# AlessioSam/LADiff

Hardware: AMD Instinct MI355X
Metric: motions/sec (196-frame, 50-step DDIM, bs128) (higher is better)
Workload: dtype f16x3+f32; 1 GPU; headline:ddim50_cfg7.5_b128_f196_c263_humanml3d; prompts_per_gpu=128, global_batch=128, frames=196, scheduler=ddim, denoising_steps=50, parallelism=dp1, loop=persistent pipeline kernel (16-row blocks x 86)

## Files before the change

### ladiff_amd/csrc/dec_mlp.hip

```cpp
#include <mutex>
#include "model.h"
#include "tile_mma.h"

namespace ladiff {

namespace {

constexpr int MLP_NS = 8;
constexpr int MLP_GRP = 4;
constexpr int MLP_STAGE = 16384;
constexpr int MLP_LDS = MLP_NS * MLP_STAGE + FF * 4 + 5 * D * 4;

typedef unsigned u32x4_m __attribute__((ext_vector_type(4)));

struct MlpArgs {
    const float* xs;
    const float* x;
    const float* w1;
    const float* b1;
    const float* w2;
    const float* b2;
    const float* g3; const float* be3;
    const float* g4; const float* be4;
    float* y; float* ys;
    int M;
};

__device__ __forceinline__ int pi_row(int p) { const int j = p >> 4, n = p & 15; return 32 * (j >> 1) + 8 * (n >> 2) + 4 * (j & 1) + (n & 3); }

template <int N> __device__ __forceinline__ void wait_vm() { asm volatile("s_waitcnt vmcnt(%0)" ::"n"(N) : "memory"); }
template <int OFF>
__device__ __forceinline__ void fetch16(u32x4_m& v, unsigned addr) {
    asm volatile("ds_read_b128 %0, %1 offset:%2" : "=v"(v) : "v"(addr), "n"(OFF) : "memory");
}
template <int OFF>
__device__ __forceinline__ void fetch16_keep(u32x4_m& v, unsigned addr) {
    asm volatile("ds_read_b128 %0, %1 offset:%2" : "+v"(v) : "v"(addr), "n"(OFF) : "memory");
}
template <int N>
__device__ __forceinline__ void wait_lgkm(u32x4_m& a, u32x4_m& b, u32x4_m& c, u32x4_m& d) {
    asm volatile("s_waitcnt lgkmcnt(%4)" : "+v"(a), "+v"(b), "+v"(c), "+v"(d) : "n"(N));
}
__device__ __forceinline__ s16x8 as_bf(const u32x4_m v) { return __builtin_bit_cast(s16x8, v); }

}

template <int NW, int RT, int DIAG = 0>
__global__ __launch_bounds__(64 * NW, NW / 4) void dec_mlp_kernel(const MlpArgs p) {
    constexpr int NT = 64 * NW, RW = 16 * RT, BM = RW * NW, PPW = 16 / NW;
    extern __shared__ __attribute__((aligned(1024))) char lds[];
    float* const b1s = reinterpret_cast<float*>(lds + MLP_NS * MLP_STAGE);
    const int tid = threadIdx.x, lane = tid & 63;
    const int wave = __builtin_amdgcn_readfirstlane(tid >> 6);
    const int frow = lane & 15, fk = lane >> 4;
    const int M = p.M;
    int myrow[RT]; bool live[RT];
#pragma unroll
    for (int rt = 0; rt < RT; ++rt) {
        myrow[rt] = blockIdx.x * BM + RW * wave + 16 * rt + frow;
        live[rt] = myrow[rt] < M;
        myrow[rt] = live[rt] ? myrow[rt] : M - 1;
    }

    s16x8 xh[RT][8], xl[RT][8];
#pragma unroll
    for (int rt = 0; rt < RT; ++rt) {
        const char* xr = reinterpret_cast<const char*>(p.xs) + (size_t)myrow[rt] * 1024 + fk * 16;
#pragma unroll
        for (int s = 0; s < 8; ++s) {
            xh[rt][s] = *reinterpret_cast<const s16x8*>(xr + (s >> 1) * 256 + (s & 1) * 64);
            xl[rt][s] = *reinterpret_cast<const s16x8*>(xr + (s >> 1) * 256 + (s & 1) * 64 + 128);
        }
    }
    for (int i = tid; i < FF / 4; i += NT) st4(b1s + 4 * i, ld4(p.b1 + 4 * i));
    float* const prm = b1s + FF;
    for (int i = tid; i < 5 * D / 4; i += NT) {
        const int which = i / (D / 4), c4 = i % (D / 4);
        const float* src = which == 0 ? p.b2 : which == 1 ? p.g3 : which == 2 ? p.be3 : which == 3 ? p.g4 : p.be4;
        if (src != nullptr) st4(prm + 4 * i, ld4(src + 4 * c4));
    }

    const int cs = (lane & 7) ^ ((lane >> 4) & 3) ^ (4 * (wave & 1));
    const int koff = (cs < 4 ? cs * 4 : 32 + (cs - 4) * 4);
    int src[PPW];
#pragma unroll
    for (int i = 0; i < PPW; ++i) src[i] = pi_row(8 * (wave + NW * i) + (lane >> 3));
    char* const dma_dst = lds + (8 * wave) * 128;
    auto issue = [&](int hs, auto uc, auto slotc, auto ic) __attribute__((always_inline)) {
        constexpr int u = decltype(uc)::value, slot = decltype(slotc)::value, i = decltype(ic)::value;
        const float* base; int ldw, n0, kb, half;
        const int hsv = hs < 0 ? 0 : hs;
        if constexpr (u < 8) { base = p.w1; ldw = D; n0 = 128 * hsv; kb = u >> 1; half = u & 1; }
        else { constexpr int v = u - 8, c = v >> 1; base = p.w2; ldw = FF; n0 = 128 * (v & 1); kb = 2 * hsv + (c >> 1); half = c & 1; }
        const float* s0 = base + (size_t)(n0 + src[i]) * ldw + kb * 64 + half * 16 + koff;
        if constexpr (DIAG == 1) { if (hs >= 0) return; }
        __builtin_amdgcn_global_load_lds(s0, (__attribute__((address_space(3))) void*)(dma_dst + slot * MLP_STAGE + 8 * NW * i * 128), 16, 0, 0);
    };

    const int sw = (frow >> 1) & 7;
    const unsigned rd_hi = lds_addr(lds) + frow * 128 + ((fk ^ sw) << 4);
    const unsigned rd_lo = lds_addr(lds) + frow * 128 + (((4 + fk) ^ sw) << 4);
    const unsigned rd_hi2 = rd_hi + 4 * MLP_STAGE, rd_lo2 = rd_lo + 4 * MLP_STAGE;

    f32x4 hacc[RT][8], oacc[RT][16];
    s16x8 hh[RT][4], hl[RT][4];
#pragma unroll
    for (int rt = 0; rt < RT; ++rt)
#pragma unroll
        for (int j = 0; j < 16; ++j) oacc[rt][j] = f32x4{0.f, 0.f, 0.f, 0.f};

    u32x4_m wt[4][2];
    u32x4_m dummy[4][2];
    if constexpr (DIAG == 3 || DIAG == 6 || DIAG == 7) {
#pragma unroll
        for (int i = 0; i < 4; ++i) { asm volatile("" : "=v"(wt[i][0])); asm volatile("" : "=v"(wt[i][1])); asm volatile("" : "=v"(dummy[i][0])); asm volatile("" : "=v"(dummy[i][1])); }
    }
    auto fetch_tile = [&](auto slotc, auto jc) __attribute__((always_inline)) {
        constexpr int slot = decltype(slotc)::value, j = decltype(jc)::value;
        if constexpr (DIAG == 3) return;
        const unsigned ah = slot < 4 ? rd_hi : rd_hi2, al = slot < 4 ? rd_lo : rd_lo2;
        constexpr int so = (slot & 3) * MLP_STAGE;
        if constexpr (DIAG == 6) { fetch16_keep<so + j * 2048>(dummy[j & 3][0], ah); fetch16_keep<so + j * 2048>(dummy[j & 3][1], al); return; }
        fetch16<so + j * 2048>(wt[j & 3][0], ah); fetch16<so + j * 2048>(wt[j & 3][1], al);
    };
    auto stage_mma = [&](auto slotc, auto& acc, auto j0c, const s16x8 (&bh)[RT], const s16x8 (&bl)[RT], auto&& between, auto&& next) __attribute__((always_inline)) {
        constexpr int slot = decltype(slotc)::value, J0 = decltype(j0c)::value;
        static_for<8>([&](auto jc) {
            constexpr int j = decltype(jc)::value, cur = j & 3;
            next(jc);
            if constexpr (DIAG != 3 && DIAG != 6) asm volatile("s_waitcnt lgkmcnt(4)" : "+v"(wt[cur][0]), "+v"(wt[cur][1]));
            __builtin_amdgcn_sched_barrier(0);
            static_for<3 * RT>([&](auto mc) {
                constexpr int m = decltype(mc)::value, prod = m / RT, rt = m % RT;
                if constexpr (DIAG == 7) {
                    acc[rt][J0 + j] = MFMA16_S16(as_bf(dummy[cur][prod == 1]), prod == 0 ? bl[rt] : bh[rt], acc[rt][J0 + j], 0, 0, 0);
                } else if constexpr (DIAG != 2) {
                    if constexpr (prod == 0) acc[rt][J0 + j] = MFMA16_S16(as_bf(wt[cur][0]), bl[rt], acc[rt][J0 + j], 0, 0, 0);
                    else if constexpr (prod == 1) acc[rt][J0 + j] = MFMA16_S16(as_bf(wt[cur][1]), bh[rt], acc[rt][J0 + j], 0, 0, 0);
                    else acc[rt][J0 + j] = MFMA16_S16(as_bf(wt[cur][0]), bh[rt], acc[rt][J0 + j], 0, 0, 0);
                }
                if constexpr (m == 0) {
                    __builtin_amdgcn_sched_barrier(0);
                    if constexpr (j + 3 < 8) fetch_tile(slotc, IntC<j + 3>{});
                    else fetch_tile(IntC<(slot + 1) % MLP_NS>{}, IntC<j + 3 - 8>{});
                    __builtin_amdgcn_sched_barrier(0);
                }
            });
            if constexpr (DIAG == 2) acc[0][J0 + j][0] += __builtin_bit_cast(float, wt[cur][0][0]) + __builtin_bit_cast(float, wt[cur][1][1]);
            __builtin_amdgcn_sched_barrier(0);
            if constexpr (j & 1) between(IntC<j / 2>{});
        });
    };

    static_for<MLP_GRP>([&](auto uc) {
        constexpr int u = decltype(uc)::value;
        static_for<PPW>([&](auto ic) { issue(DIAG == 1 ? -1 : 0, IntC<u>{}, IntC<u>{}, ic); });
    });
    __syncthreads();
    auto landed = [&]() __attribute__((always_inline)) {
        wait_vm<0>();
        __builtin_amdgcn_s_barrier();
    };
    landed();
    static_for<PPW>([&](auto ic) { issue(DIAG == 1 ? -1 : 0, IntC<MLP_GRP>{}, IntC<MLP_GRP>{}, ic); });
    static_for<3>([&](auto jc) { fetch_tile(IntC<0>{}, jc); });
    constexpr int H = PPW / 2;
#pragma unroll 1
    for (int hs = 0; hs < 8; ++hs) {
        static_for<16>([&](auto uc) {
            constexpr int u = decltype(uc)::value, slot = u % MLP_NS, r = u % MLP_GRP;
            auto batch_pieces = [&](auto aheadc, auto halfc) __attribute__((always_inline)) {
                constexpr int ahead = decltype(aheadc)::value, half = decltype(halfc)::value;
                constexpr int ut = (u + ahead) % 16, slot_t = (u + ahead) % MLP_NS;
                const int hs_t = (hs + (u + ahead >= 16 ? 1 : 0)) & 7;
                static_for<H>([&](auto ic) { issue(hs_t, IntC<ut>{}, IntC<slot_t>{}, IntC<H * half + decltype(ic)::value>{}); });
            };
            auto between = [&](auto gc) __attribute__((always_inline)) {
                constexpr int g = decltype(gc)::value;
                if constexpr (r == 3 && g >= 2) batch_pieces(IntC<5>{}, IntC<g - 2>{});
                else if constexpr (r == 0 && g < 2) batch_pieces(IntC<5>{}, IntC<g>{});
                else if constexpr (r == 0 && g >= 2) batch_pieces(IntC<6>{}, IntC<g - 2>{});
                else if constexpr (r == 1 && g < 2) batch_pieces(IntC<6>{}, IntC<g>{});
            };
            auto next = [&](auto jc) __attribute__((always_inline)) {
                constexpr int j = decltype(jc)::value;
                if constexpr (r == 3 && j == 5) landed();
                else if constexpr (r == 0 && j == 5) __builtin_amdgcn_s_barrier();
            };
            if constexpr (u < 8) {
                if constexpr (u == 0) {
#pragma unroll
                    for (int rt = 0; rt < RT; ++rt)
#pragma unroll
                        for (int j = 0; j < 8; ++j) hacc[rt][j] = f32x4{0.f, 0.f, 0.f, 0.f};
                }
                s16x8 bh[RT], bl[RT];
#pragma unroll
                for (int rt = 0; rt < RT; ++rt) { bh[rt] = xh[rt][u]; bl[rt] = xl[rt][u]; }
                stage_mma(IntC<slot>{}, hacc, IntC<0>{}, bh, bl, between, next);
            } else {
                constexpr int v = u - 8, c = v >> 1, nh = v & 1;
                if constexpr (nh == 0) {
                    const f32x4 ba = ld4(b1s + 128 * hs + 32 * c + 8 * fk), bb = ld4(b1s + 128 * hs + 32 * c + 8 * fk + 4);
#pragma unroll
                    for (int rt = 0; rt < RT; ++rt) {
                        f32x4 va, vb;
#pragma unroll
                        for (int e = 0; e < 4; ++e) {
                            if constexpr (DIAG == 4) { va[e] = hacc[rt][2 * c][e] + ba[e]; vb[e] = hacc[rt][2 * c + 1][e] + bb[e]; }
                            else { va[e] = gelu_erf(hacc[rt][2 * c][e] + ba[e]); vb[e] = gelu_erf(hacc[rt][2 * c + 1][e] + bb[e]); }
                        }
                        split8(va, vb, hh[rt][c], hl[rt][c]);
                    }
                }
                s16x8 bh[RT], bl[RT];
#pragma unroll
                for (int rt = 0; rt < RT; ++rt) { bh[rt] = hh[rt][c]; bl[rt] = hl[rt][c]; }
                stage_mma(IntC<slot>{}, oacc, IntC<8 * nh>{}, bh, bl, between, next);
            }
        });
    }
    wait_vm<0>();
    if constexpr (DIAG == 6) {
        wait_lgkm<0>(dummy[0][0], dummy[0][1], dummy[1][0], dummy[1][1]);
        wait_lgkm<0>(dummy[2][0], dummy[2][1], dummy[3][0], dummy[3][1]);
    } else if constexpr (DIAG != 3) {
        wait_lgkm<0>(wt[0][0], wt[0][1], wt[1][0], wt[1][1]);
        wait_lgkm<0>(wt[2][0], wt[2][1], wt[3][0], wt[3][1]);
    }

    if constexpr (DIAG == 5) {
        float s = 0.f;
#pragma unroll
        for (int rt = 0; rt < RT; ++rt)
#pragma unroll
            for (int jj = 0; jj < 16; ++jj) s += oacc[rt][jj][0] + oacc[rt][jj][1] + oacc[rt][jj][2] + oacc[rt][jj][3];
        if (live[0] && p.y != nullptr) p.y[(size_t)myrow[0] * D + fk] = s;
        return;
    }
    __syncthreads();
    char* const stg = lds + wave * 16384;
#pragma unroll
    for (int rt = 0; rt < RT; ++rt) {
        const size_t rbase = (size_t)myrow[rt] * D;
        f32x4 (&v)[16] = oacc[rt];
        float s = 0.f;
#pragma unroll
        for (int jj = 0; jj < 16; ++jj) {
            const int col = 32 * (jj >> 1) + 8 * fk + 4 * (jj & 1);
            const f32x4 bv = ld4(prm + col), rv = ld4(p.x + rbase + col);
#pragma unroll
            for (int e = 0; e < 4; ++e) { v[jj][e] = v[jj][e] + bv[e] + rv[e]; }
            s += (v[jj][0] + v[jj][1]) + (v[jj][2] + v[jj][3]);
        }
#pragma unroll
        for (int pass = 0; pass < 2; ++pass) {
            if (pass == 1 && p.g4 == nullptr) break;
            const float* gp = prm + (pass == 0 ? 1 : 3) * D;
            const float* bp = prm + (pass == 0 ? 2 : 4) * D;
            if (pass == 1) {
                s = 0.f;
#pragma unroll
                for (int jj = 0; jj < 16; ++jj) s += (v[jj][0] + v[jj][1]) + (v[jj][2] + v[jj][3]);
            }
            s += __shfl_xor(s, 16, 64); s += __shfl_xor(s, 32, 64);
            const float mean = s * (1.f / 256.f);
            float q = 0.f;
#pragma unroll
            for (int jj = 0; jj < 16; ++jj)
#pragma unroll
                for (int e = 0; e < 4; ++e) { const float d = v[jj][e] - mean; q = fmaf(d, d, q); }
            q += __shfl_xor(q, 16, 64); q += __shfl_xor(q, 32, 64);
            const float rstd = rsqrtf(q * (1.f / 256.f) + LN_EPS);
#pragma unroll
            for (int jj = 0; jj < 16; ++jj) {
                const int col = 32 * (jj >> 1) + 8 * fk + 4 * (jj & 1);
                const f32x4 ga = ld4(gp + col), be = ld4(bp + col);
#pragma unroll
                for (int e = 0; e < 4; ++e) v[jj][e] = (v[jj][e] - mean) * rstd * ga[e] + be[e];
            }
        }
#pragma unroll
        for (int jj = 0; jj < 16; ++jj) {
            const int ch = 8 * (jj >> 1) + 2 * fk + (jj & 1);
            *reinterpret_cast<f32x4*>(stg + frow * 1024 + ((ch ^ frow) << 4)) = v[jj];
        }
        const int row0 = blockIdx.x * BM + RW * wave + 16 * rt;
#pragma unroll
        for (int r = 0; r < 16; ++r) {
            const f32x4 o = *reinterpret_cast<const f32x4*>(stg + r * 1024 + ((lane ^ r) << 4));
            if (row0 + r < M) {
                if (p.y != nullptr) st4(p.y + (size_t)(row0 + r) * D + 4 * lane, o);
                if (p.ys != nullptr) store_split4(p.ys + (size_t)(row0 + r) * D, 4 * lane, o);
            }
        }
    }
}

std::atomic<int> g_mlp_variant{0};

int dec_mlp_prepare() {
    static std::mutex mu;
    static bool attr_set[64] = {};
    int dev = 0;
    LADIFF_HIP(hipGetDevice(&dev));
    if (dev < 0 || dev >= 64) return LADIFF_ERR_ARG;
    std::lock_guard<std::mutex> lock(mu);
    if (!attr_set[dev]) {
        const void* k[3] = {reinterpret_cast<const void*>(dec_mlp_kernel<4, 2>), reinterpret_cast<const void*>(dec_mlp_kernel<8, 1>),
                            reinterpret_cast<const void*>(dec_mlp_kernel<4, 1>)};
        for (int i = 0; i < 3; ++i) LADIFF_HIP(hipFuncSetAttribute(k[i], hipFuncAttributeMaxDynamicSharedMemorySize, MLP_LDS));
#ifdef LADIFF_STAMPS
        const void* d[7] = {reinterpret_cast<const void*>(dec_mlp_kernel<4, 2, 1>), reinterpret_cast<const void*>(dec_mlp_kernel<4, 2, 2>),
                            reinterpret_cast<const void*>(dec_mlp_kernel<4, 2, 3>), reinterpret_cast<const void*>(dec_mlp_kernel<4, 2, 4>),
                            reinterpret_cast<const void*>(dec_mlp_kernel<4, 2, 5>), reinterpret_cast<const void*>(dec_mlp_kernel<4, 2, 6>),
                            reinterpret_cast<const void*>(dec_mlp_kernel<4, 2, 7>)};
        for (int i = 0; i < 7; ++i) LADIFF_HIP(hipFuncSetAttribute(d[i], hipFuncAttributeMaxDynamicSharedMemorySize, MLP_LDS));
#endif
        attr_set[dev] = true;
    }
    return 0;
}
int dec_mlp_min_rows() { return 10000; }

int launch_dec_mlp(const float* xs, const float* x, const float* w1, const float* b1, const float* w2, const float* b2, const float* g3,
                   const float* be3, const float* g4, const float* be4, float* y, float* ys, int M, hipStream_t s) {
    if (M <= 0) return 0;
    LADIFF_TRY(dec_mlp_prepare());
    MlpArgs a{xs, x, w1, b1, w2, b2, g3, be3, g4, be4, y, ys, M};
    int form = g_mlp_variant;
    if (form >= 21) form = 0;
    if (form == 0) form = (M + 127) / 128 < 160 ? 2 : 1;
#ifdef LADIFF_STAMPS
    if (form >= 11 && form <= 17) {
        const void* k[7] = {reinterpret_cast<const void*>(dec_mlp_kernel<4, 2, 1>), reinterpret_cast<const void*>(dec_mlp_kernel<4, 2, 2>),
                            reinterpret_cast<const void*>(dec_mlp_kernel<4, 2, 3>), reinterpret_cast<const void*>(dec_mlp_kernel<4, 2, 4>),
                            reinterpret_cast<const void*>(dec_mlp_kernel<4, 2, 5>), reinterpret_cast<const void*>(dec_mlp_kernel<4, 2, 6>),
                            reinterpret_cast<const void*>(dec_mlp_kernel<4, 2, 7>)};
        void* args[] = {&a};
        LADIFF_HIP(hipLaunchKernel(k[form - 11], dim3((M + 127) / 128), dim3(256), args, MLP_LDS, s));
    } else
#endif
    if (form == 3) hipLaunchKernelGGL((dec_mlp_kernel<4, 2>), dim3((M + 127) / 128), dim3(256), MLP_LDS, s, a);
    else if (form == 1) hipLaunchKernelGGL((dec_mlp_kernel<8, 1>), dim3((M + 127) / 128), dim3(512), MLP_LDS, s, a);
    else hipLaunchKernelGGL((dec_mlp_kernel<4, 1>), dim3((M + 63) / 64), dim3(256), MLP_LDS, s, a);
    LADIFF_LAUNCH_CHECK();
    return 0;
}

}
```

Baseline: 11310 motions/s.

## Interleave GELU epilogue and bias loads into MFMA stage slots

Moves the bias-add, GELU and hi/lo split of the first FFN layer out of a serial block at the start of each second-layer chunk. The work is now spread across the MFMA loop of the preceding stages through a hook, so VALU work overlaps matrix-core work. Bias values are read with inline ds_read_b128 into registers ahead of use. This adds register pressure and a complex per-(u,j) schedule that is easy to get wrong, and any error would show up as wrong outputs rather than a build failure.

New measurement: 11340 motions/s, median of 6. No clear change (+0.3%).

```diff
diff --git a/ladiff_amd/csrc/dec_mlp.hip b/ladiff_amd/csrc/dec_mlp.hip
--- a/ladiff_amd/csrc/dec_mlp.hip
+++ b/ladiff_amd/csrc/dec_mlp.hip
@@ -123,7 +123,8 @@
         if constexpr (DIAG == 6) { fetch16_keep<so + j * 2048>(dummy[j & 3][0], ah); fetch16_keep<so + j * 2048>(dummy[j & 3][1], al); return; }
         fetch16<so + j * 2048>(wt[j & 3][0], ah); fetch16<so + j * 2048>(wt[j & 3][1], al);
     };
-    auto stage_mma = [&](auto slotc, auto& acc, auto j0c, const s16x8 (&bh)[RT], const s16x8 (&bl)[RT], auto&& between, auto&& next) __attribute__((always_inline)) {
+    auto stage_mma = [&](auto slotc, auto& acc, auto j0c, const s16x8 (&bh)[RT], const s16x8 (&bl)[RT], auto&& between, auto&& next,
+                         auto&& vwork) __attribute__((always_inline)) {
         constexpr int slot = decltype(slotc)::value, J0 = decltype(j0c)::value;
         static_for<8>([&](auto jc) {
             constexpr int j = decltype(jc)::value, cur = j & 3;
@@ -141,8 +142,11 @@
                 }
                 if constexpr (m == 0) {
                     __builtin_amdgcn_sched_barrier(0);
+                    vwork(jc, IntC<0>{});
                     if constexpr (j + 3 < 8) fetch_tile(slotc, IntC<j + 3>{});
                     else fetch_tile(IntC<(slot + 1) % MLP_NS>{}, IntC<j + 3 - 8>{});
+                    __builtin_amdgcn_sched_barrier(0);
+                    vwork(jc, IntC<1>{});
                     __builtin_amdgcn_sched_barrier(0);
                 }
             });
@@ -165,6 +169,8 @@
     static_for<PPW>([&](auto ic) { issue(DIAG == 1 ? -1 : 0, IntC<MLP_GRP>{}, IntC<MLP_GRP>{}, ic); });
     static_for<3>([&](auto jc) { fetch_tile(IntC<0>{}, jc); });
     constexpr int H = PPW / 2;
+    u32x4_m gb[2];
+    const unsigned b1_rd = lds_addr(b1s) + 32 * fk;
 #pragma unroll 1
     for (int hs = 0; hs < 8; ++hs) {
         static_for<16>([&](auto uc) {
@@ -187,6 +193,43 @@
                 if constexpr (r == 3 && j == 5) landed();
                 else if constexpr (r == 0 && j == 5) __builtin_amdgcn_s_barrier();
             };
+            auto gelu_hook = [&](auto jc, auto phc) __attribute__((always_inline)) {
+                constexpr int j = decltype(jc)::value, ph = decltype(phc)::value;
+                if constexpr (ph == 0) {
+                    constexpr int n = u - 6;
+                    constexpr int bc = u == 7 ? (j == 0 || j == 4 ? 0 : j == 6 ? 1 : -1) : (u >= 8 && u <= 12 && j == 6 ? (n + 1) >> 1 : -1);
+                    constexpr int bhf = u == 7 ? (j == 4 ? 1 : 0) : ((n & 1) ^ 1);
+                    if constexpr (bc >= 0)
+                        asm volatile("ds_read_b128 %0, %1 offset:%2" : "=v"(gb[bhf]) : "v"(b1_rd + 512u * hs), "n"(128 * bc + 16 * bhf) : "memory");
+                } else {
+                    constexpr int gc = u == 7 ? 0 : (u >= 8 && u <= 13 ? (u - 6) >> 1 : -1);
+                    constexpr int k0 = u == 7 ? (j < 2 ? 0 : j < 6 ? j - 2 : 2 * j - 8) : (j & 1 ? 0 : 4 * (u & 1) + j / 2);
+                    constexpr int k1 = u == 7 ? (j < 2 ? 0 : j < 6 ? j - 1 : 2 * j - 6) : (j & 1 ? 0 : k0 + 1);
+                    constexpr int sh = (u == 7 && j == 5) ? 0 : (u == 7 && j == 7) ? 1 : (u != 7 && j == 6) ? (u & 1) : -1;
+                    if constexpr (gc >= 0 && k1 > k0) {
+                        if constexpr (DIAG == 3 || DIAG == 6) asm volatile("s_waitcnt lgkmcnt(0)" ::: "memory");
+                        asm volatile("" : "+v"(gb[k0 >> 2]));
+                        const f32x4 bq = __builtin_bit_cast(f32x4, gb[k0 >> 2]);
+                        static_for<k1 - k0>([&](auto ic) {
+                            constexpr int k = k0 + decltype(ic)::value, a = 2 * gc + (k >> 2), e = k & 3;
+#pragma unroll
+                            for (int rt = 0; rt < RT; ++rt) {
+                                if constexpr (DIAG == 4) hacc[rt][a][e] = hacc[rt][a][e] + bq[e];
+                                else hacc[rt][a][e] = gelu_erf(hacc[rt][a][e] + bq[e]);
+                            }
+                        });
+                        if constexpr (sh >= 0) {
+#pragma unroll
+                            for (int rt = 0; rt < RT; ++rt) {
+                                s16x4 hi4, lo4;
+                                split4(hacc[rt][2 * gc + sh], hi4, lo4);
+#pragma unroll
+                                for (int e = 0; e < 4; ++e) { hh[rt][gc][4 * sh + e] = hi4[e]; hl[rt][gc][4 * sh + e] = lo4[e]; }
+                            }
+                        }
+                    }
+                }
+            };
             if constexpr (u < 8) {
                 if constexpr (u == 0) {
 #pragma unroll
@@ -197,26 +240,13 @@
                 s16x8 bh[RT], bl[RT];
 #pragma unroll
                 for (int rt = 0; rt < RT; ++rt) { bh[rt] = xh[rt][u]; bl[rt] = xl[rt][u]; }
-                stage_mma(IntC<slot>{}, hacc, IntC<0>{}, bh, bl, between, next);
+                stage_mma(IntC<slot>{}, hacc, IntC<0>{}, bh, bl, between, next, gelu_hook);
             } else {
                 constexpr int v = u - 8, c = v >> 1, nh = v & 1;
-                if constexpr (nh == 0) {
-                    const f32x4 ba = ld4(b1s + 128 * hs + 32 * c + 8 * fk), bb = ld4(b1s + 128 * hs + 32 * c + 8 * fk + 4);
-#pragma unroll
-                    for (int rt = 0; rt < RT; ++rt) {
-                        f32x4 va, vb;
-#pragma unroll
-                        for (int e = 0; e < 4; ++e) {
-                            if constexpr (DIAG == 4) { va[e] = hacc[rt][2 * c][e] + ba[e]; vb[e] = hacc[rt][2 * c + 1][e] + bb[e]; }
-                            else { va[e] = gelu_erf(hacc[rt][2 * c][e] + ba[e]); vb[e] = gelu_erf(hacc[rt][2 * c + 1][e] + bb[e]); }
-                        }
-                        split8(va, vb, hh[rt][c], hl[rt][c]);
-                    }
-                }
                 s16x8 bh[RT], bl[RT];
 #pragma unroll
                 for (int rt = 0; rt < RT; ++rt) { bh[rt] = hh[rt][c]; bl[rt] = hl[rt][c]; }
-                stage_mma(IntC<slot>{}, oacc, IntC<8 * nh>{}, bh, bl, between, next);
+                stage_mma(IntC<slot>{}, oacc, IntC<8 * nh>{}, bh, bl, between, next, gelu_hook);
             }
         });
     }
```
